# AVianEco/Softspoken

Hardware: AMD Instinct MI355X
Metric: audio-seconds processed/sec (whole node), 16 kHz mono (higher is better)
Workload: dtype f16x2

## Files before the change

### softspoken_amd/csrc/conv4.hip

```cpp
#include "kernels.h"
#include <cstdio>
#include <cstdlib>
#include <type_traits>
#include <utility>

namespace ss {

#ifdef SS_DEVBUILD
static int dev_env(const char* name, int dflt) { const char* v = getenv(name); return v ? atoi(v) : dflt; }
#else
static constexpr int dev_env(const char*, int dflt) { return dflt; }
#endif

typedef float f32x16 __attribute__((ext_vector_type(16)));
typedef float f32x4 __attribute__((ext_vector_type(4)));
typedef float f32x2 __attribute__((ext_vector_type(2)));
typedef __bf16 bf16x8 __attribute__((ext_vector_type(8)));
typedef __bf16 bf16x2 __attribute__((ext_vector_type(2)));
typedef _Float16 f16x8 __attribute__((ext_vector_type(8)));
typedef _Float16 f16x2 __attribute__((ext_vector_type(2)));
typedef short s16x2 __attribute__((ext_vector_type(2)));
typedef uint32_t u32x4 __attribute__((ext_vector_type(4)));
typedef uint32_t u32x2 __attribute__((ext_vector_type(2)));

// ... 5 lines not shown

__device__ __forceinline__ void lds_barrier4() { asm volatile("s_waitcnt lgkmcnt(0)\n\ts_barrier" ::: "memory"); }

__device__ __forceinline__ uint32_t pack_bf16(float lo, float hi) {
    return __builtin_bit_cast(uint32_t, __builtin_convertvector(f32x2{lo, hi}, bf16x2));
}
__device__ __forceinline__ uint32_t relu_pk(uint32_t v) {
    return __builtin_bit_cast(uint32_t, __builtin_elementwise_max(__builtin_bit_cast(s16x2, v), s16x2{0, 0}));
}
__device__ __forceinline__ uint32_t max_pk(uint32_t a, uint32_t b) {
    return __builtin_bit_cast(uint32_t, __builtin_elementwise_max(__builtin_bit_cast(s16x2, a), __builtin_bit_cast(s16x2, b)));
}
__device__ __forceinline__ uint32_t pack_f16(float lo, float hi) {
    return __builtin_bit_cast(uint32_t, __builtin_convertvector(f32x2{lo, hi}, f16x2));
}
__device__ __forceinline__ f32x2 unpack_f16(uint32_t v) { return __builtin_convertvector(__builtin_bit_cast(f16x2, v), f32x2); }
__device__ __forceinline__ uint32_t pk_max_u16(uint32_t a, uint32_t b) {
    uint32_t r;
    asm("v_pk_max_u16 %0, %1, %2" : "=v"(r) : "v"(a), "v"(b));
    return r;
}
__device__ __forceinline__ uint32_t split_lo(uint32_t hi, float x0, float x1) {
    uint32_t l;
    asm("v_fma_mixlo_f16 %0, %1, -1.0, %2 op_sel_hi:[1,0,0]" : "=v"(l) : "v"(hi), "v"(x0));
    asm("v_fma_mixhi_f16 %0, %1, -1.0, %2 op_sel:[1,0,0] op_sel_hi:[1,0,0]" : "+v"(l) : "v"(hi), "v"(x1));
    return l;
}
template <bool F16>
__device__ __forceinline__ f32x16 mfma16(const u32x4& a, const u32x4& b, const f32x16& c) {
    if constexpr (F16) return __builtin_amdgcn_mfma_f32_32x32x16_f16(__builtin_bit_cast(f16x8, a), __builtin_bit_cast(f16x8, b), c, 0, 0, 0);
    else return __builtin_amdgcn_mfma_f32_32x32x16_bf16(__builtin_bit_cast(bf16x8, a), __builtin_bit_cast(bf16x8, b), c, 0, 0, 0);
}
__device__ __forceinline__ void half_swap(uint32_t& x, uint32_t& y) {
    const u32x2 r = __builtin_amdgcn_permlane32_swap(x, y, false, false);
    x = r[0]; y = r[1];
}

struct Packed { uint32_t p[4][2]; };

__device__ __forceinline__ void to_runs(Packed& k, u32x4& lo, u32x4& hi) {
    half_swap(k.p[0][0], k.p[1][0]); half_swap(k.p[0][1], k.p[1][1]);
    half_swap(k.p[2][0], k.p[3][0]); half_swap(k.p[2][1], k.p[3][1]);
    lo = u32x4{k.p[0][0], k.p[0][1], k.p[1][0], k.p[1][1]};
    hi = u32x4{k.p[2][0], k.p[2][1], k.p[3][0], k.p[3][1]};
}
__device__ __forceinline__ void from_runs(const u32x4& lo, const u32x4& hi, Packed& k) {
    k.p[0][0] = lo[0]; k.p[0][1] = lo[1]; k.p[1][0] = lo[2]; k.p[1][1] = lo[3];
    k.p[2][0] = hi[0]; k.p[2][1] = hi[1]; k.p[3][0] = hi[2]; k.p[3][1] = hi[3];
    half_swap(k.p[0][0], k.p[1][0]); half_swap(k.p[0][1], k.p[1][1]);
    half_swap(k.p[2][0], k.p[3][0]); half_swap(k.p[2][1], k.p[3][1]);
}

template <int NT, int NW, bool BRES, bool RES, bool RADD, bool POOL, int RP, bool FIRST, bool FLAT, bool PF2, bool SPLIT = false, bool RANK1 = false,
          int NH = 1>
__global__ __launch_bounds__(64 * NW * NH) __attribute__((amdgpu_waves_per_eu((NT <= 2 && !(SPLIT && RES && !BRES && NW == 4 && NH == 1)) ? 4 : 2)))
void conv3x3_v4_kernel(ConvArgs a, int total_tiles, int lds_b_bytes) {
    constexpr int KC = 32;
    constexpr bool DUO = NH > 1;
    static_assert(!DUO || (NT == 1 && NW * NH == 16 && RP == 0 && !FIRST && !FLAT && !PF2), "DUO: the plain A / B launches");
    constexpr bool RING = DUO && !BRES;
    static_assert(!RING || (SPLIT && NH == 4), "RING: f16x2, four 4-wave tiles");
    static_assert(!SPLIT || !PF2, "SPLIT: single-stage prefetch");
    static_assert(!RANK1 || (SPLIT && !RES && !RADD), "RANK1: conv1_1.B in f16x2 mode");
    static_assert(!(FIRST && SPLIT) || RANK1, "FIRST in f16x2 mode: the block's residual is the fp32 rank-1 term");
    static_assert(!FLAT || (NT == 1 && NW == 8 && BRES && (RADD || RP) && !POOL && !FIRST), "FLAT: conv9_1.B");
    static_assert(!PF2 || (BRES && !FIRST), "two-stage prefetch: resident-weight launches");
    static_assert(RP == 0 || (!RES && !RADD && !FIRST), "RP: a B launch that computes the block's projection itself (no r tensor)");
    static_assert(!FIRST || (NT == 1 && BRES && !RES && !RADD), "FIRST: conv1_1.B, one 32 -> 32 chunk, rank-1 residual");
    constexpr int kTapBytes = 2 * NT * 1024;
    constexpr int TAPS = RES ? 10 : 9;
    constexpr int NTHR = 64 * NW;
    constexpr int TH = 2 * NW;
    constexpr int PR = TH + 2;
    constexpr int kA = PR * kRowPitch;
    constexpr int NPA = PR * kPatch * 4;
    constexpr int AIT = (NPA + NTHR - 1) / NTHR;
    constexpr int NPB = (SPLIT ? 2 : 1) * TAPS * kTapBytes / 16;
    constexpr int BIT = BRES ? 1 : (DUO ? (NPB / 2 + NTHR - 1) / NTHR : (NPB + NTHR - 1) / NTHR);
    static_assert(!(RES && (RADD || POOL)), "RES is the A launch; RADD / POOL belong to B launches");
    static_assert(AIT <= 4, "edge flags are packed 8 bits per piece");
    extern __shared__ __attribute__((aligned(16))) char smem[];

    const int half = DUO ? __builtin_amdgcn_readfirstlane((int)threadIdx.x / NTHR) : 0;
    const int tid = DUO ? (int)threadIdx.x % NTHR : (int)threadIdx.x, lane = tid & 63;
    const int wave = __builtin_amdgcn_readfirstlane(tid >> 6);
    const int hh = lane >> 5, m = lane & 31;
    const int py = (m >> 1) & 1, px = (m & 1) | ((m >> 2) << 1);
    char* sA = smem + half * kA;
    const int sb_bytes = RING ? 2 * lds_b_bytes : lds_b_bytes;
    char* sB = smem + NH * kA;
    const int proj_steps = RP ? (a.C0x + a.C1x) / 16 : 0;
    constexpr bool proj_lds = RP > 0 && (BRES || NT == 3 || SPLIT);
    const char* sProj = smem + NH * kA + sb_bytes;
    const int proj_tiles = SPLIT ? a.Cout / 32 : NT;
    const int proj_bank = proj_steps * proj_tiles * 1024;
    const float* sBias = (const float*)(sProj + (proj_lds ? (SPLIT ? 2 : 1) * proj_bank : 0));
    constexpr int FW = 20, FROWS = PR + 3;
    float* sFb = (float*)sBias + 32;
    float* sF = sFb + 32;
    float* sFlat = (float*)sBias + 32;

    const int H = a.H, W = a.W, Cout = a.Cout;
    const int ngroups = Cout / (32 * NT);
    const int nch_r = (a.C0 + a.C1) / KC;
    const int nch = SPLIT ? 2 * nch_r : nch_r;
    const int all_taps = nch_r * TAPS;

    const int xcd = blockIdx.x & 7, local = (int)(blockIdx.x >> 3) * NH + half, gper = (int)(gridDim.x >> 3) * NH;
    const int per = (total_tiles + 7) >> 3;
#ifdef SS_DEVBUILD
    const bool order_seq = !(a.dbg & 512);
#else
    constexpr bool order_seq = !kOrderSideBySide;
#endif
    auto tile_of = [&](int loc, int it) -> int {
        if constexpr (RING) {
            const RingItem r = ring_item(xcd, loc / NH, (int)(gridDim.x >> 3), it, loc % NH, total_tiles / ngroups, ngroups, order_seq);
            return r.pos >= 0 ? r.pos * ngroups + r.g : -1;
        }
        const int idx = loc + it * gper;
        const int t = xcd * per + idx;
        return (idx < per && t < total_tiles) ? t : -1;
    };
    auto tile_at = [&](int it) -> int { return tile_of(local, it); };
    struct Tile { int n, y0, x0, g; };
    auto decode = [&](int t) -> Tile {
        Tile d;
        d.g = t % ngroups; t /= ngroups;
        d.x0 = (t % a.tiles_x) * 16; t /= a.tiles_x;
        d.y0 = (t % a.tiles_y) * TH;
        d.n = t / a.tiles_y;
        return d;
    };

    uint32_t pix_full[AIT], pix_half[AIT], lds_off[AIT], flags = 0;
    const uint32_t part16 = (tid & 3) * 16;
    {
        const int Wh = W >> 1;
#pragma unroll
        for (int it = 0; it < AIT; ++it) {
            const int p = tid + NTHR * it;
            const int pix = p >> 2;
            const int pyy = pix / kPatch, pxx = pix - pyy * kPatch;
            lds_off[it] = pyy * kRowPitch + pxx * kPixPitch + part16;
            pix_full[it] = pyy * W + pxx;
            pix_half[it] = ((pyy + 1) >> 1) * Wh + ((pxx + 1) >> 1);
            const uint32_t f = (pyy == 0 ? 1u : 0u) | (pyy == PR - 1 ? 2u : 0u) | (pxx == 0 ? 4u : 0u) | (pxx == kPatch - 1 ? 8u : 0u) |
                               (p >= NPA ? 16u : 0u);
            flags |= f << (8 * it);
        }
    }
    u32x4 ra0[AIT], ra1[AIT];
    u32x4 rb[BIT];
    float rf = 0.f;
    static_assert(!FIRST || (PR + 2) * FW <= NTHR, "one feature value per thread");

    auto issue_patch = [&](const Tile& d, int ci, u32x4 (&ra)[AIT]) {
        if constexpr (FIRST) {
            if constexpr (SPLIT) { if (ci & 1) return; }
            const int fy = tid / FW, fx = tid - fy * FW;
            const int Y = d.y0 - 2 + fy, X = d.x0 - 2 + fx;
            rf = (tid < (PR + 2) * FW && (unsigned)Y < (unsigned)H && (unsigned)X < (unsigned)W)
                     ? a.rank1_src[((size_t)d.n * H + Y) * W + X] : 0.f;
            return;
        }
        const int ch = (SPLIT ? ci >> 1 : ci) * KC;
        const int64_t plane = (SPLIT && !(ci & 1)) ? a.lo_delta : 0;
        const char* base; uint32_t cs2, toff; bool up;
// ... 65 lines not shown
                    if (p < NPH) v = *(const u32x4*)(wsrc + p * 16);
                    rb[it] = v;
                }
            } else {
                char* dst = sB + (k & 1) * lds_b_bytes + half * (TAPS * kTapBytes);
#pragma unroll
                for (int it = 0; it < BIT; ++it) {
                    const int p = tid + NTHR * it;
                    if (p < NPH) *(u32x4*)(dst + p * 16) = rb[it];
                }
            }
        }
    };

    constexpr int RPH = RP >= 2 ? RP / 2 : RP;
    u32x4 pxh[(SPLIT && RP) ? RPH : 1], pxl[(SPLIT && RP) ? RPH : 1];
    auto issue_proj = [&](const Tile& d, int chunk, auto k0c, auto k1c) {
        constexpr int K0 = decltype(k0c)::value, K1 = decltype(k1c)::value;
        if constexpr (SPLIT && RP > 0 && K1 > K0) {
            const uint32_t t_full = kHdr + ((((uint32_t)d.n * H + d.y0 + 2 * wave) * W + d.x0) * a.C0x) * 2u;
            const uint32_t t_half = kHdr + ((((uint32_t)d.n * (H >> 1) + (d.y0 >> 1) + wave) * (W >> 1) + (d.x0 >> 1)) * a.C1x) * 2u;
            uint32_t zl = 0;
            asm volatile("" : "+v"(zl));
            const uint32_t xf_o = (uint32_t)((py * W + px) * a.C0x + hh * 8) * 2u + zl, xh_o = (uint32_t)((px >> 1) * a.C1x + hh * 8) * 2u + zl;
#pragma unroll
            for (int k = K0; k < K1; ++k) {
                const int sidx = chunk * RP + k, ch = sidx * 16;
                const char* base; uint32_t off;
                if (sidx >= proj_steps) { base = (const char*)a.xp0 - kHdr; off = 0; }
                else if (ch < a.C0x) { base = (const char*)a.xp0 - kHdr; off = t_full + xf_o + ch * 2u; }
                else { base = (const char*)a.xp1 - kHdr; off = t_half + xh_o + (ch - a.C0x) * 2u; }
                pxh[k - K0] = *(const u32x4*)(base + off);
                pxl[k - K0] = *(const u32x4*)(base + a.lo_delta + off);
            }
        }
    };

    int it_tile = 0;
    struct Stage { int ci; Tile d; };
    auto next_stage = [&](const Stage& s0, Stage& n) -> bool {
        n = s0; n.ci = s0.ci + 1;
        if (n.ci == nch) {
            n.ci = 0;
            const int t = tile_at(++it_tile);
            if (t < 0) return false;
            n.d = decode(t);
        }
        return true;
    };
    int my_stages = 0, max_stages = 0;
    if constexpr (DUO) {
        const int l0 = (int)(blockIdx.x >> 3) * NH;
        int n0 = 0, nmine = 0;
        while (tile_of(l0, n0) >= 0) ++n0;
        while (tile_of(l0 + half, nmine) >= 0) ++nmine;
        my_stages = nmine * nch;
        max_stages = n0 * nch;
        if (max_stages == 0) return;
    } else {
        if (tile_at(0) < 0) return;
    }
    Stage cs{0, decode((DUO && my_stages == 0) ? 0 : tile_at(0))}, n1 = cs, n2 = cs;

    if constexpr (BRES || RING) {
        const char* wsrc = (const char*)a.wpk + (RING ? (size_t)ring_g0 * nch_r * 2 * (TAPS * kTapBytes) : 0);
        for (int p = tid; p < lds_b_bytes / 16; p += NTHR) *(u32x4*)(sB + p * 16) = *(const u32x4*)(wsrc + (size_t)p * 16);
    }
    for (int i = tid; i < Cout * (RES ? 2 : 1); i += NTHR)
        ((float*)sBias)[i] = i < Cout ? a.bias[i] : a.res_bias[i - Cout];
    if constexpr (proj_lds)
        for (int p = tid; p < (SPLIT ? 2 : 1) * proj_steps * proj_tiles * 64; p += NTHR) *(u32x4*)((char*)sProj + p * 16) = *(const u32x4*)((const char*)a.proj_w + (size_t)p * 16);
    u32x4 wfirst = {0u, 0u, 0u, 0u}, wr1 = {0u, 0u, 0u, 0u}, wfirst_lo = {0u, 0u, 0u, 0u};
    constexpr int NMT = (PR * kPatch + 31) / 32;
    int pf_off[2], pa_off[2]; uint32_t pflags = 0;
    if constexpr (FIRST) {
        for (int i = tid; i < 32; i += NTHR) sFb[i] = a.first_b[i];
        for (int i = tid; i < FROWS * FW; i += NTHR) sF[i] = 0.f;
        const float* w9 = a.first_w;
        auto wv = [&](int t) { return w9[t * 32 + m]; };
        if constexpr (SPLIT) {
            auto hi2 = [&](float x, float y) { return pack_f16(x, y); };
            auto lo2 = [&](float x, float y) { const f32x2 b = unpack_f16(pack_f16(x, y)); return pack_f16(x - b[0], y - b[1]); };
            if (hh == 0) {
                wfirst = u32x4{hi2(wv(0), wv(1)), hi2(wv(2), 0.f), hi2(wv(3), wv(4)), hi2(wv(5), 0.f)};
                wfirst_lo = u32x4{lo2(wv(0), wv(1)), lo2(wv(2), 0.f), lo2(wv(3), wv(4)), lo2(wv(5), 0.f)};
            } else {
                wfirst = u32x4{hi2(wv(6), wv(7)), hi2(wv(8), 0.f), 0u, 0u};
                wfirst_lo = u32x4{lo2(wv(6), wv(7)), lo2(wv(8), 0.f), 0u, 0u};
            }
        } else if (hh == 0) {
            wfirst = u32x4{pack_bf16(wv(0), wv(1)), pack_bf16(wv(2), 0.f), pack_bf16(wv(3), wv(4)), pack_bf16(wv(5), 0.f)};
            const float w = a.rank1_w[m];
            const float whi = (float)(__bf16)w, wlo = w - whi;
            wr1 = u32x4{pack_bf16(whi, whi), pack_bf16(wlo, 0.f), 0u, 0u};
        } else {
            wfirst = u32x4{pack_bf16(wv(6), wv(7)), pack_bf16(wv(8), 0.f), 0u, 0u};
        }
#pragma unroll
        for (int t = 0; t < 2; ++t) {
            const int q = 32 * (wave + NW * t) + m;
            const bool in = q < PR * kPatch;
            const int qq = in ? q : 0;
            const int qy = qq / kPatch, qx = qq - qy * kPatch;
            pf_off[t] = (qy + 2 * hh) * FW + qx;
            pa_off[t] = qy * kRowPitch + qx * kPixPitch + hh * 16;
            const uint32_t f = (qy == 0 ? 1u : 0u) | (qy == PR - 1 ? 2u : 0u) | (qx == 0 ? 4u : 0u) | (qx == kPatch - 1 ? 8u : 0u) | (in ? 0u : 16u);
            pflags |= f << (8 * t);
        }
    }
    u32x4 hk_lo[(FIRST && SPLIT) ? 2 : 1], hk_hi[(FIRST && SPLIT) ? 2 : 1];
    auto produce = [&](const Tile& d, int part) {
        const uint32_t tm = (d.y0 == 0 ? 1u : 0u) | (d.y0 + TH == H ? 2u : 0u) | (d.x0 == 0 ? 4u : 0u) | (d.x0 + 16 == W ? 8u : 0u) | 16u;
#pragma unroll
        for (int t = 0; t < 2; ++t) {
            if (wave + NW * t < NMT) {
                if constexpr (SPLIT) {
                    if (part) {
// ... 169 lines not shown
                else { base = (const char*)a.xp1 - kHdr; off = t_half + xh_off + (ch - a.C0x) * 2u; }
                xf[k] = *(const u32x4*)(base + off);
            }
        }
        u32x4 wpg[(RP && !proj_lds) ? RP : 1][NT];
        if constexpr (RP > 0 && !proj_lds && !SPLIT) {
            {
                const int tiles = Cout / 32;
#pragma unroll
                for (int k = 0; k < RP; ++k) {
                    const int sidx = ci * RP + k < proj_steps ? ci * RP + k : 0;
#pragma unroll
                    for (int nt = 0; nt < NT; ++nt)
                        wpg[k][nt] = *(const u32x4*)((const char*)a.proj_w + ((size_t)(sidx * tiles + cur.g * NT + nt) * 64 + lane) * 16);
                }
            }
        }
        if (ci == 0) {
#pragma unroll
            for (int nt = 0; nt < NT; ++nt)
#pragma unroll
                for (int g = 0; g < 4; ++g) {
                    const f32x4 b4 = *(const f32x4*)(sBias + co0 + nt * 32 + 8 * g + 4 * hh);
                    acc[nt][4 * g] = b4[0]; acc[nt][4 * g + 1] = b4[1]; acc[nt][4 * g + 2] = b4[2]; acc[nt][4 * g + 3] = b4[3];
                    if constexpr (RES) {
                        const f32x4 r4 = *(const f32x4*)(sBias + Cout + co0 + nt * 32 + 8 * g + 4 * hh);
                        racc[nt][4 * g] = r4[0]; racc[nt][4 * g + 1] = r4[1]; racc[nt][4 * g + 2] = r4[2]; racc[nt][4 * g + 3] = r4[3];
                    }
                }
        }
        auto proj_products = [&](auto k0c, auto k1c) {
            constexpr int K0 = decltype(k0c)::value, K1 = decltype(k1c)::value;
#pragma unroll
            for (int k = K0; k < K1; ++k) {
                const int sidx = (ci >> 1) * RP + k < proj_steps ? (ci >> 1) * RP + k : 0;
#pragma unroll
                for (int nt = 0; nt < NT; ++nt) {
                    const int wt = (sidx * proj_tiles + (int)(co0 >> 5) + nt) * 1024 + lane * 16;
                    const u32x4 wh = *(const u32x4*)(sProj + wt), wl = *(const u32x4*)(sProj + proj_bank + wt);
                    acc[nt] = mfma16<true>(wh, pxl[k - K0], acc[nt]);
                    acc[nt] = mfma16<true>(wl, pxh[k - K0], acc[nt]);
                    acc[nt] = mfma16<true>(wh, pxh[k - K0], acc[nt]);
                }
            }
        };
        using KZ_ = std::integral_constant<int, 0>; using KH_ = std::integral_constant<int, RPH>; using KR_ = std::integral_constant<int, RP>;
        if constexpr (SPLIT && RP > 0 && PART == 1) {
            proj_products(KZ_{}, KH_{});
            __builtin_amdgcn_sched_barrier(0);
            if constexpr (RP > RPH) issue_proj(cur, ci >> 1, KH_{}, KR_{});
        }
        if constexpr (FLAT && SPLIT && RP > 0) load_flat_w();
        {
            const char* bbase = sB + boff0 + (BRES ? ((DUO ? cur.g * nch : 0) + (SPLIT ? (ci >> 1) * 2 : ci)) * TAPS * kTapBytes
                                                   : RING ? ((stage_no >> 1) & 1) * lds_b_bytes : 0);
            constexpr int PD = (NT == 1) ? 4 : 2;
            u32x4 af[PD], bfr[PD][NT];
            u32x4 rfr[RES ? 2 : 1][RES ? NT : 1];
            if (a.dbg & 32) __builtin_amdgcn_s_setprio(kMfmaPrio);
            constexpr bool kMerged = SPLIT && NSTEP == 36 && NT == 1;
            if constexpr (kMerged) {
                constexpr int PM = 3;
                u32x4 pf[PM], wh_[PM], wl_[PM], rh_[RES ? 2 : 1], rl_[RES ? 2 : 1];
                const char* bb0 = bbase; const char* bb1 = bbase + TAPS * kTapBytes;
                auto load3 = [&](int st, int slot) {
                    const int tap = st >> 1, sub = st & 1, dy = tap / 3, dx = tap % 3;
                    pf[slot] = *(const u32x4*)(sA + aoff0 + dy * kRowPitch + dx * kPixPitch + sub * 32);
                    wh_[slot] = *(const u32x4*)(bb0 + tap * kTapBytes + sub * 1024);
                    wl_[slot] = *(const u32x4*)(bb1 + tap * kTapBytes + sub * 1024);
                };
#pragma unroll
                for (int st = 0; st < PM - 1; ++st) load3(st, st);
#pragma unroll
                for (int st = 0; st < 18; ++st) {
                    if (st + PM - 1 < 18) load3(st + PM - 1, (st + PM - 1) % PM);
                    if constexpr (RES) {
                        if (st == 6) {
#pragma unroll
                            for (int sub = 0; sub < 2; ++sub) {
                                rh_[sub] = *(const u32x4*)(bb0 + 9 * kTapBytes + sub * 1024);
                                rl_[sub] = *(const u32x4*)(bb1 + 9 * kTapBytes + sub * 1024);
                            }
                        }
                    }
                    const u32x4 pixv = pf[st % PM];
                    acc[0] = mfma16<true>(wh_[st % PM], pixv, acc[0]);
                    acc[0] = mfma16<true>(wl_[st % PM], pixv, acc[0]);
                    if constexpr (RES) {
                        if (st == 8 || st == 9) {
                            racc[0] = mfma16<true>(rh_[st & 1], pixv, racc[0]);
                            racc[0] = mfma16<true>(rl_[st & 1], pixv, racc[0]);
                        }
                    }
                }
            } else
#pragma unroll
            for (int bank = 0; bank < NSTEP / 18; ++bank) {
                const char* bb = bbase + bank * TAPS * kTapBytes;
                auto load_frags = [&](int st, u32x4& fa, u32x4 (&fbb)[NT]) {
                    const int tap = st >> 1, sub = st & 1, dy = tap / 3, dx = tap % 3;
                    fa = *(const u32x4*)(sA + aoff0 + dy * kRowPitch + dx * kPixPitch + sub * 32);
#pragma unroll
                    for (int nt = 0; nt < NT; ++nt) fbb[nt] = *(const u32x4*)(bb + tap * kTapBytes + (sub * NT + nt) * 1024);
                };
                if (bank) __builtin_amdgcn_sched_barrier(0);
#pragma unroll
                for (int st = 0; st < PD - 1; ++st) load_frags(st, af[st], bfr[st]);
// ... 228 lines not shown
    #pragma unroll
                            for (int h = 0; h < 2; ++h) {
                                uint32_t v = k.p[g][h];
                                v = max_pk(v, (uint32_t)__builtin_amdgcn_mov_dpp((int)v, 0xB1, 0xf, 0xf, true));
                                v = max_pk(v, (uint32_t)__builtin_amdgcn_mov_dpp((int)v, 0x4E, 0xf, 0xf, true));
                                kp.p[g][h] = v;
                            }
                    }
                    u32x4 lo, hi;
                    if (!FLAT || a.store_out) {
                        to_runs(k, lo, hi);
                        *(u32x4*)(op + nt * 64) = lo;
                        *(u32x4*)(op + nt * 64 + 32) = hi;
                    }
                    if constexpr (RES) {
                        Packed kr;
    #pragma unroll
                        for (int g = 0; g < 4; ++g)
    #pragma unroll
                            for (int h = 0; h < 2; ++h) kr.p[g][h] = pack_bf16(racc[nt][4 * g + 2 * h], racc[nt][4 * g + 2 * h + 1]);
                        to_runs(kr, lo, hi);
                        char* rp = (char*)a.res_out + (o_tile + st_off);
                        *(u32x4*)(rp + nt * 64) = lo;
                        *(u32x4*)(rp + nt * 64 + 32) = hi;
                    }
                    if constexpr (POOL) {
                        to_runs(kp, lo, hi);
                        const u32x4 pv = (m & 1) ? hi : lo;
                        if ((m & 3) < 2) {
                            const uint32_t p_tile = ((((uint32_t)cur.n * (H >> 1) + (cur.y0 >> 1) + wave) * (W >> 1) + (cur.x0 >> 1)) * Cout + co0) * 2u;
                            char* pp = (char*)a.pool_out + (p_tile + pl_off);
                            *(u32x4*)(pp + nt * 64 + (m & 1) * 32) = pv;
                        }
                    }
                }
            }
        };
        constexpr bool EPI_EARLY = PF2;
        jitter(1);
        if constexpr (EPI_EARLY) epilogue();
        lds_barrier4();
        jitter(2);
#ifdef SS_DEVBUILD
        uint32_t tw_i = 0;
#endif
        if constexpr (DUO) {
            if (ok1) {
                commit(ra_a, kCommitPatch, kCommitBank);
                ok2 = next_stage(n1, n2);
                if (ok2) { issue_patch(n2.d, n2.ci, ra_a); issue_weights(n2.d, n2.ci); }
            }
            ring_duty(stage_no, max_stages >> 1);
            ++stage_no;
            jitter(4);
            epilogue();
            jitter(6);
            lds_barrier4();
            jitter(5);
            cs = n1; n1 = n2;
            const bool more = ok1;
            ok1 = ok1 && ok2;
            return more;
        }
        if constexpr (FLAT) { if (flat_pending) flat_reduce(flat_tile); }
        if (ok1) {
            if constexpr (FIRST) {
                if constexpr (!SPLIT || NEXT == 0) {
                    if (tid < (PR + 2) * FW) sF[tid] = rf;
                    lds_barrier4();
                }
                jitter(3);
                produce(n1.d, NEXT);
            } else {
#ifdef SS_DEVBUILD
                uint32_t tw0 = 0;
                if (a.stamps) { tw0 = (uint32_t)__builtin_amdgcn_s_memtime(); asm volatile("s_waitcnt vmcnt(0)" ::: "memory"); const uint32_t t = (uint32_t)__builtin_amdgcn_s_memtime(); st_sum[5] += t - tw0; tw0 = t; }
#endif
                commit(ra_a, kCommitPatch, kCommitBank);
#ifdef SS_DEVBUILD
                if (a.stamps) { asm volatile("s_waitcnt lgkmcnt(0)" ::: "memory"); const uint32_t t = (uint32_t)__builtin_amdgcn_s_memtime(); st_sum[6] += t - tw0; tw_i = t; }
#endif
            }
            if constexpr (PF2) {
                ok3 = ok2 && next_stage(n2, n3);
                if (ok3) issue_patch(n3.d, n3.ci, ra_a);
            } else {
                ok2 = next_stage(n1, n2);
#ifdef SS_DEVBUILD
                if (a.stamps) { const uint32_t t = (uint32_t)__builtin_amdgcn_s_memtime(); st_sum[7] += t - tw_i; tw_i = t; }
#endif
                if (ok2) issue_patch(n2.d, n2.ci, ra_a);
#ifdef SS_DEVBUILD
                if (a.stamps) { const uint32_t t = (uint32_t)__builtin_amdgcn_s_memtime(); st_sum[8] += t - tw_i; tw_i = t;
                                const uint32_t t2 = (uint32_t)__builtin_amdgcn_s_memtime(); st_sum[9] += t2 - t; }
#endif
            }
            if (ok2) issue_weights(n2.d, n2.ci);
            if constexpr (SPLIT && RP > 0 && PART == 0) issue_proj(cur, ci >> 1, KZ_{}, KH_{});
            jitter(4);
            lds_barrier4();
        } else if constexpr (FLAT) {
            lds_barrier4();
        }
        jitter(5);
        if constexpr (!EPI_EARLY) epilogue();
        if constexpr (FLAT) { flat_pending = last; flat_tile = cur; }
        if (!ok1) {
            if constexpr (FLAT) { lds_barrier4(); if (flat_pending) flat_reduce(flat_tile); }
            return false;
        }
        cs = n1; n1 = n2; ok1 = ok2;
        if constexpr (PF2) { n2 = n3; ok2 = ok3; }
        return true;
    };
    using P0 = std::integral_constant<int, 0>; using P1 = std::integral_constant<int, 1>;
    if constexpr (DUO) {
        for (int i = 0; i < half; ++i) lds_barrier4();
        for (int s = 0; s < max_stages; s += SPLIT ? 2 : 1) {
            if (s < my_stages) {
                stage(P0{}, ra0);
                if constexpr (SPLIT) stage(P1{}, ra0);
            } else {
                lds_barrier4(); ring_duty(s, max_stages >> 1); lds_barrier4();
                if constexpr (SPLIT) { lds_barrier4(); ring_duty(s + 1, max_stages >> 1); lds_barrier4(); }
            }
        }
        for (int i = half; i < NH - 1; ++i) lds_barrier4();
    } else if constexpr (SPLIT) {
        while (stage(P0{}, ra0) && stage(P1{}, ra0)) {}
    } else if constexpr (PF2) {
        while (stage(P0{}, ra0) && stage(P0{}, ra1)) {}
    } else {
        while (stage(P0{}, ra0)) {}
    }
#ifdef SS_DEVBUILD
    if (a.stamps && lane == 0) {
        uint32_t* p = (uint32_t*)a.stamps + (((size_t)blockIdx.x * NH + half) * NW + wave) * 16;
        for (int i = 0; i < 5; ++i) p[i] = st_sum[i];
        p[5] = (uint32_t)jit_n; p[6] = st_sum[5]; p[7] = st_sum[6]; p[8] = st_sum[7]; p[9] = st_sum[8]; p[10] = st_sum[9]; p[11] = st_sum[10]; p[12] = st_sum[11];
    }
#endif
}

template <int NT, int NW, bool BRES, bool RES, bool RADD, bool POOL, int RP, bool FIRST, bool FLAT, bool PF2, bool SPLIT = false, bool RANK1 = false,
          int NH = 1>
static hipError_t launch_v4_k(const ConvArgs& a, int total, int lds_b, size_t lds, int grid, hipStream_t s) {
    static std::atomic<uint64_t> attr_done{0};
    if (hipError_t e = allow_full_lds((const void*)conv3x3_v4_kernel<NT, NW, BRES, RES, RADD, POOL, RP, FIRST, FLAT, PF2, SPLIT, RANK1, NH>, attr_done)) return e;
    hipLaunchKernelGGL((conv3x3_v4_kernel<NT, NW, BRES, RES, RADD, POOL, RP, FIRST, FLAT, PF2, SPLIT, RANK1, NH>), dim3(grid), dim3(64 * NW * NH),
                       lds, s, a, total, lds_b);
    return hipGetLastError();
}

template <int NW, int NH, bool BRES>
static hipError_t launch_v4_duo(const ConvArgs& a, int total, int lds_b, size_t lds, int grid, hipStream_t s) {
    if constexpr (BRES && NH == 4) {
        if (a.plain) return launch_v4_k<1, NW, true, false, false, false, 0, false, false, false, true, false, NH>(a, total, lds_b, lds, grid, s);
    }
    if (a.res_out) return launch_v4_k<1, NW, BRES, true, false, false, 0, false, false, false, true, false, NH>(a, total, lds_b, lds, grid, s);
    if (a.pool_out) return launch_v4_k<1, NW, BRES, false, true, true, 0, false, false, false, true, false, NH>(a, total, lds_b, lds, grid, s);
    return launch_v4_k<1, NW, BRES, false, true, false, 0, false, false, false, true, false, NH>(a, total, lds_b, lds, grid, s);
}

template <int NT, int NW>
static hipError_t launch_v4_split(const ConvArgs& a, bool bres, int total, int lds_b, size_t lds, int grid, hipStream_t s) {
    if constexpr (NT == 1 && NW == 8) {
        if (a.rank1_src && a.first_w) return launch_v4_k<1, 8, true, false, false, true, 0, true, false, false, true, true>(a, total, lds_b, lds, grid, s);
        if (a.rank1_src) return launch_v4_k<1, 8, true, false, false, true, 0, false, false, false, true, true>(a, total, lds_b, lds, grid, s);
        if (a.flat_part && a.proj_w) return launch_v4_k<1, 8, true, false, false, false, 4, false, true, false, true>(a, total, lds_b, lds, grid, s);
        if (a.flat_part) return launch_v4_k<1, 8, true, false, true, false, 0, false, true, false, true>(a, total, lds_b, lds, grid, s);
        if (a.proj_w) return bres ? hipErrorInvalidValue : launch_v4_k<1, 8, false, false, false, true, 1, false, false, false, true>(a, total, lds_b, lds, grid, s);
    }
    if (a.res_out) return bres ? launch_v4_k<NT, NW, true, true, false, false, 0, false, false, false, true>(a, total, lds_b, lds, grid, s)
                               : launch_v4_k<NT, NW, false, true, false, false, 0, false, false, false, true>(a, total, lds_b, lds, grid, s);
    if (a.pool_out) return bres ? launch_v4_k<NT, NW, true, false, true, true, 0, false, false, false, true>(a, total, lds_b, lds, grid, s)
                                : launch_v4_k<NT, NW, false, false, true, true, 0, false, false, false, true>(a, total, lds_b, lds, grid, s);
    return bres ? launch_v4_k<NT, NW, true, false, true, false, 0, false, false, false, true>(a, total, lds_b, lds, grid, s)
                : launch_v4_k<NT, NW, false, false, true, false, 0, false, false, false, true>(a, total, lds_b, lds, grid, s);
}

static bool v4_pf2(bool bres, size_t lds, int NT, bool first, bool flat) {
    static const int env = dev_env("SOFTSPOKEN_PF2", 1);
    return env && bres && !first && !flat && NT <= 2 && lds * 3 > 160 * 1024;
}

template <int NT, int NW, bool BRES, bool RES, bool RADD, bool POOL, int RP = 0, bool FIRST = false, bool FLAT = false>
static hipError_t launch_v4_t(const ConvArgs& a, int total, int lds_b, size_t lds, int grid, hipStream_t s) {
    if constexpr (BRES && !FIRST && !FLAT && RP == 0 && NT <= 2 && NW == 8 && !(RES && NT == 2)) {
        if (v4_pf2(true, lds, NT, false, false)) return launch_v4_k<NT, NW, BRES, RES, RADD, POOL, RP, FIRST, FLAT, true>(a, total, lds_b, lds, grid, s);
    }
    return launch_v4_k<NT, NW, BRES, RES, RADD, POOL, RP, FIRST, FLAT, false>(a, total, lds_b, lds, grid, s);
}

static int v4_rp(const ConvArgs& a) {
    if (!a.proj_w) return 0;
    const int steps = (a.C0x + a.C1x) / 16, nch = (a.C0 + a.C1) / 32;
    const int per = (steps + nch - 1) / nch;
    return per <= 1 ? 1 : per <= 2 ? 2 : per <= 4 ? 4 : per <= 6 ? 6 : -1;
}

template <int NT, int NW>
static hipError_t launch_v4_kind(const ConvArgs& a, bool bres, int total, int lds_b, size_t lds, int grid, hipStream_t s) {
    const int rp = v4_rp(a);
    if constexpr (NT == 1 && NW == 8) {
        if (a.first_w) return launch_v4_t<1, 8, true, false, false, true, 0, true>(a, total, lds_b, lds, grid, s);
        if (a.flat_part) return rp == 4 ? launch_v4_t<1, 8, true, false, false, false, 4, false, true>(a, total, lds_b, lds, grid, s)
                                        : launch_v4_t<1, 8, true, false, true, false, 0, false, true>(a, total, lds_b, lds, grid, s);
    }
    if (rp) {
        if constexpr (NT == 2 && NW == 8) { if (bres && a.pool_out && rp == 1) return launch_v4_t<2, 8, true, false, false, true, 1>(a, total, lds_b, lds, grid, s); }
        if constexpr (NT == 3 && NW == 8) { if (!bres && a.pool_out && rp == 2) return launch_v4_t<3, 8, false, false, false, true, 2>(a, total, lds_b, lds, grid, s); }
        if constexpr (NT == 2 && NW == 8) { if (!bres && a.pool_out && rp == 2) return launch_v4_t<2, 8, false, false, false, true, 2>(a, total, lds_b, lds, grid, s); }
        if constexpr (NT == 1 && NW == 4) { if (!bres && !a.pool_out && rp == 2) return launch_v4_t<1, 4, false, false, false, false, 2>(a, total, lds_b, lds, grid, s); }
        if constexpr (NT == 2 && NW == 8) { if (bres && !a.pool_out && rp == 6) return launch_v4_t<2, 8, true, false, false, false, 6>(a, total, lds_b, lds, grid, s); }
        return hipErrorInvalidValue;
    }
    if (a.plain) return bres ? launch_v4_t<NT, NW, true, false, false, false>(a, total, lds_b, lds, grid, s)
                             : launch_v4_t<NT, NW, false, false, false, false>(a, total, lds_b, lds, grid, s);
    if (a.res_out) return bres ? launch_v4_t<NT, NW, true, true, false, false>(a, total, lds_b, lds, grid, s)
                               : launch_v4_t<NT, NW, false, true, false, false>(a, total, lds_b, lds, grid, s);
    if (a.pool_out) return bres ? launch_v4_t<NT, NW, true, false, true, true>(a, total, lds_b, lds, grid, s)
                                : launch_v4_t<NT, NW, false, false, true, true>(a, total, lds_b, lds, grid, s);
    return bres ? launch_v4_t<NT, NW, true, false, true, false>(a, total, lds_b, lds, grid, s)
                : launch_v4_t<NT, NW, false, false, true, false>(a, total, lds_b, lds, grid, s);
}

#ifndef SS_RPROJ_DEFAULT
#define SS_RPROJ_DEFAULT 2
#endif
#ifndef SS_DUO_DEFAULT
#define SS_DUO_DEFAULT 4
#endif
struct V4Choice { bool ok; int nw, total, lds_b, grid; bool bres; size_t lds; int duo; };

static V4Choice choose_v4(ConvArgs& a, int NT, int num_cus, int prec) {
    V4Choice c{};
    if (prec != 1 && prec != 2) return c;
    const bool split = prec == 2;
    if (!a.relu || a.R0 || a.R1) return c;
    const bool first = a.first_w != nullptr, flat = a.flat_part != nullptr, proj = a.proj_w != nullptr;
    const bool rank1 = split && a.rank1_src != nullptr;
    if (split) {
        if (a.lo_delta <= 0) return c;
        static const int rproj_env = dev_env("SOFTSPOKEN_RPROJ", SS_RPROJ_DEFAULT);
        if (proj && !(NT == 1 && a.H % 16 == 0 && ((flat && v4_rp(a) == 4 && rproj_env == 2) || (!flat && a.pool_out && a.Cout == 64 && v4_rp(a) == 1)))) return c;
        if (first && !rank1) return c;
        if (rank1 && !(NT == 1 && a.rank1_w && a.pool_out && !a.res_out && !a.res_in && !flat && a.C0 == 32 && a.C1 == 0 && a.H % 16 == 0)) return c;
        if (NT == 2 || !(NT == 1 || (a.H % 16 == 0))) return c;
    }
    const int rp = v4_rp(a);
    if (flat && !(NT == 1 && a.Cout == 32 && a.C0 == 32 && a.C1 == 0 && a.H % 16 == 0 && a.flat_w4 && (a.res_in || rp == 4) && !a.pool_out && !first)) return c;
    if (first) {
        if (!(NT == 1 && a.Cout == 32 && a.C0 == 32 && a.C1 == 0 && a.H % 16 == 0 && a.first_b && a.rank1_src && a.rank1_w && a.pool_out &&
              !a.res_out && !a.res_in && !proj && !a.plain)) return c;
    } else if (proj) {
        if (a.rank1_src || a.res_out || a.res_in || a.plain || rp < 0 || !a.xp0 || a.C0x % 16 || a.C1x % 16 || (a.C1x && !a.xp1)) return c;
        if (a.C0 != a.Cout || a.C1 != 0) return c;
        if ((double)a.N * a.H * a.W * std::max(a.C0x, a.C1x) * 2.0 + kHdr >= 4294967296.0) return c;
    } else if (a.plain) {
        if (a.rank1_src || a.res_out || a.res_in || a.pool_out) return c;
    } else if (!rank1) {
        if (a.rank1_src) return c;
        if (!(a.res_out || a.res_in) || (a.res_out && (a.res_in || a.pool_out))) return c;
    }
    if (a.W % 16 != 0 || a.H % 8 != 0 || a.Cout % (32 * NT) != 0 || NT < 1 || NT > 3) return c;
    if (a.C0 % 32 || a.C1 % 32 || (a.C1 && ((a.H | a.W) & 1))) return c;
    if ((double)a.N * a.H * a.W * std::max(a.Cout, std::max(a.C0, a.C1)) * 2.0 + kHdr >= 4294967296.0) return c;
    c.nw = (a.H % 16 == 0) ? 8 : 4;
    const int th = 2 * c.nw;
    a.tiles_y = a.H / th; a.tiles_x = a.W / 16;
    const int ngroups = a.Cout / (32 * NT);
    const long total_l = (long)a.N * a.tiles_y * a.tiles_x * ngroups;
    if (total_l <= 0 || total_l > 0x7fffffff) return c;
    c.total = (int)total_l;
    const int tap_bytes = 2 * NT * 1024;
    const int taps = a.res_out ? 10 : 9;
    const int all_taps = ((a.C0 + a.C1) / 32) * taps;
    static const int bres_kb = dev_env("SOFTSPOKEN_BRES_KB", 72);
    const int banks = split ? 2 : 1;
    c.bres = ngroups == 1 && (size_t)all_taps * tap_bytes * banks <= (size_t)((first || flat || rank1) ? 72 : bres_kb) * 1024;
    c.lds_b = c.bres ? all_taps * tap_bytes * banks : taps * tap_bytes * banks;
    if ((first || flat || rank1) && !c.bres) return c;
    if (proj && !flat && !((NT == 2 && c.nw == 8 && c.bres && a.pool_out && rp == 1) ||
                           (NT == 3 && c.nw == 8 && !c.bres && ngroups == 1 && a.pool_out && rp == 2) ||
                           (NT == 2 && c.nw == 8 && !c.bres && ngroups > 1 && a.pool_out && rp == 2) ||
                           (NT == 1 && c.nw == 4 && !c.bres && ngroups > 1 && !a.pool_out && rp == 2) ||
                           (split && NT == 1 && c.nw == 8 && !c.bres && ngroups > 1 && a.pool_out && rp == 1) ||
                           (NT == 2 && c.nw == 8 && c.bres && !a.pool_out && rp == 6)))
        return c;
    static const int duo_env = dev_env("SOFTSPOKEN_DUO", SS_DUO_DEFAULT);
    static const int duo8_env = dev_env("SOFTSPOKEN_DUO_H8", 1);
    if ((duo_env == 2 || duo_env == 4) && split && NT == 1 && (c.nw == 8 || (duo_env == 4 && duo8_env)) && !first && !flat && !proj && !rank1) {
        const int nh = duo_env, thd = 32 / nh;
        const size_t fixed = nh * (size_t)(thd + 2) * kRowPitch + (size_t)a.Cout * 4 * (a.res_out ? 2 : 1);
        const size_t chunk_b = (size_t)taps * tap_bytes * banks;
        const size_t all_b = (size_t)ngroups * all_taps * tap_bytes * banks;
        const bool bres = fixed + all_b <= 160 * 1024;
        static const int ring_env = dev_env("SOFTSPOKEN_RING", 1);
        const bool ring = !bres && nh == 4 && ring_env && (a.res_out != nullptr || ring_env == 2 || (a.H <= 32 && a.res_in != nullptr));
        const size_t lds = fixed + (bres ? all_b : 2 * chunk_b);
        if (((bres && (!a.plain || nh == 4)) || (ring && !a.plain)) && lds <= 160 * 1024) {
            c.duo = nh; c.bres = bres; c.lds_b = (int)(bres ? all_b : chunk_b); c.lds = lds;
            c.nw = 16 / nh;
            a.tiles_y = a.H / thd;
            c.total = (int)((long)a.N * a.tiles_y * a.tiles_x * ngroups);
            c.grid = (num_cus + 7) / 8 * 8;
            if (c.grid * nh > c.total) c.grid = ((c.total + nh - 1) / nh + 7) / 8 * 8;
            c.ok = true;
            return c;
        }
    }
    if (split && a.plain) return c;
    c.lds = (size_t)(th + 2) * kRowPitch + c.lds_b + (size_t)a.Cout * 4 * (a.res_out ? 2 : 1) + (first ? (size_t)(32 + (th + 5) * 20) * 4 : 0) +
            (flat ? (size_t)c.nw * 2 * 64 * 4 : 0) + (proj && (ngroups == 1 || split) ? (size_t)((a.C0x + a.C1x) / 16) * (split ? a.Cout / 32 : NT) * 1024 * banks : 0);
    int bpc = (int)((160 * 1024) / c.lds);
    if (bpc < 1) return c;
    if (bpc > 3) bpc = 3;
    { static const int cap = dev_env("SOFTSPOKEN_BPC", 3); if (bpc > cap) bpc = cap; }
    c.grid = num_cus * bpc;
    if (c.grid > c.total) c.grid = c.total;
    c.grid = (c.grid + 7) / 8 * 8;
    c.ok = true;
    return c;
}

int conv_v4_flat_groups() { return 128 / 16; }

bool conv_v4_supports(const ConvArgs& a_in, int NT, int num_cus, int prec) {
    ConvArgs a = a_in;
    return choose_v4(a, NT, num_cus, prec).ok;
}

const char* conv_v4_variant(const ConvArgs& a_in, int NT, int num_cus, int prec) {
    static thread_local char buf[112];
    ConvArgs a = a_in;
    const V4Choice c = choose_v4(a, NT, num_cus, prec);
    if (!c.ok) return "conv3x3_v4_kernel<invalid>";
    auto tf = [](bool b) { return b ? "true" : "false"; };
    const bool res = a.res_out != nullptr, first = a.first_w != nullptr, flat = a.flat_part != nullptr;
    const int rp = v4_rp(a);
    const bool split = prec == 2, rank1 = split && a.rank1_src != nullptr;
    const bool radd = !res && !first && !a.plain && rp == 0 && !rank1;
    const bool pf2 = !split && rp == 0 && c.nw == 8 && !(res && NT == 2) && v4_pf2(c.bres, c.lds, NT, first, flat);
    if (split)
        snprintf(buf, sizeof buf, "conv3x3_v4_kernel<%d, %d, %s, %s, %s, %s, %d, %s, %s, false, true, %s, %d>", NT, c.nw, tf(c.bres), tf(res), tf(radd),
                 tf(!res && a.pool_out), rp, tf(first), tf(flat), tf(rank1), c.duo ? c.duo : 1);
    else
        snprintf(buf, sizeof buf, "conv3x3_v4_kernel<%d, %d, %s, %s, %s, %s, %d, %s, %s, %s, false, false, 1>", NT, c.nw, tf(c.bres), tf(res), tf(radd),
                 tf(!res && a.pool_out), rp, tf(first), tf(flat), tf(pf2));
    return buf;
}

hipError_t launch_conv3x3_v4(const ConvArgs& a_in, int NT, int num_cus, int prec, hipStream_t s) {
    ConvArgs a = a_in;
    const V4Choice c = choose_v4(a, NT, num_cus, prec);
    if (!c.ok) return hipErrorInvalidValue;
    if (prec == 2) {
        if (c.duo == 2) return launch_v4_duo<8, 2, true>(a, c.total, c.lds_b, c.lds, c.grid, s);
        if (c.duo == 4) return c.bres ? launch_v4_duo<4, 4, true>(a, c.total, c.lds_b, c.lds, c.grid, s)
                                      : launch_v4_duo<4, 4, false>(a, c.total, c.lds_b, c.lds, c.grid, s);
        if (c.nw == 8) {
            switch (NT) {
                case 1: return launch_v4_split<1, 8>(a, c.bres, c.total, c.lds_b, c.lds, c.grid, s);
                case 3: return launch_v4_split<3, 8>(a, c.bres, c.total, c.lds_b, c.lds, c.grid, s);
            }
        } else if (NT == 1) return launch_v4_split<1, 4>(a, c.bres, c.total, c.lds_b, c.lds, c.grid, s);
        return hipErrorInvalidValue;
    }
    if (c.nw == 8) {
        switch (NT) {
            case 1: return launch_v4_kind<1, 8>(a, c.bres, c.total, c.lds_b, c.lds, c.grid, s);
            case 2: return launch_v4_kind<2, 8>(a, c.bres, c.total, c.lds_b, c.lds, c.grid, s);
            case 3: return launch_v4_kind<3, 8>(a, c.bres, c.total, c.lds_b, c.lds, c.grid, s);
        }
    } else {
        switch (NT) {
            case 1: return launch_v4_kind<1, 4>(a, c.bres, c.total, c.lds_b, c.lds, c.grid, s);
            case 2: return launch_v4_kind<2, 4>(a, c.bres, c.total, c.lds_b, c.lds, c.grid, s);
            case 3: return launch_v4_kind<3, 4>(a, c.bres, c.total, c.lds_b, c.lds, c.grid, s);
        }
    }
    return hipErrorInvalidValue;
}

}
```

### softspoken_amd/csrc/kernels.h

```cpp
#pragma once
#include <hip/hip_runtime.h>
#include <stdint.h>
#include <atomic>

namespace ss {

inline hipError_t allow_full_lds(const void* kernel, std::atomic<uint64_t>& done) {
    int dev = 0;
    hipError_t e = hipGetDevice(&dev);
    if (e != hipSuccess) return e;
    const uint64_t bit = 1ull << (dev & 63);
    if (done.load(std::memory_order_acquire) & bit) return hipSuccess;
    e = hipFuncSetAttribute(kernel, hipFuncAttributeMaxDynamicSharedMemorySize, 160 * 1024);
    if (e == hipSuccess) done.fetch_or(bit, std::memory_order_release);
    return e;
}

struct ConvArgs {
    const void* src0; const void* src1;
    const void* res0; const void* res1;
    const void* wpk;
    const float* bias;
    const float* rank1_src;
    const float* rank1_w;
    void* out;
    void* pool_out;
    int N, H, W, C0, C1, R0, R1, Cout;
    int relu;
    int tiles_y, tiles_x;
    int dbg;
    const float* first_w; const float* first_b;
    const void* flat_w; float* flat_part;
    int store_out;
    const void* flat_w4;
    void* res_out; const float* res_bias;
    const void* res_in;
    const void* wpk_b; const float* bias_a;
    int plain;
    const void* proj_w;
    const void* xp0; const void* xp1; int C0x, C1x;
    int64_t lo_delta;
    int* range_flag;
    void* stamps;
};
static constexpr bool kOrderSideBySide = true;
struct RingItem { int pos, g; };
__host__ __device__ inline int ring_lim(int xcd, int total_pos) {
    const int per_pos = (total_pos + 7) >> 3, left = total_pos - xcd * per_pos;
    return left < 0 ? 0 : left < per_pos ? left : per_pos;
}
__host__ __device__ inline int ring_group0(int wg, int ngroups, bool seq) { return seq ? 0 : wg % ngroups; }
__host__ __device__ inline int ring_group_step(int G, int ngroups, bool seq) { return seq ? 1 % ngroups : G % ngroups; }
__host__ __device__ inline RingItem ring_item(int xcd, int wg, int G, int item, int tile, int total_pos, int ngroups, bool seq) {
    const int lim = ring_lim(xcd, total_pos);
    int quad, g;
    if (seq) { quad = wg + (item / ngroups) * G; g = item % ngroups; }
    else { const int j = wg + item * G; quad = j / ngroups; g = j - quad * ngroups; }
    const int idx = 4 * quad + tile;
    return RingItem{idx < lim ? xcd * ((total_pos + 7) >> 3) + idx : -1, g};
}
__host__ __device__ inline int ring_items(int xcd, int wg, int G, int tile, int total_pos, int ngroups, bool seq) {
    const int lim = ring_lim(xcd, total_pos);
    const int quads = lim > tile ? (lim - tile + 3) >> 2 : 0;
    if (seq) return quads > wg ? (quads - wg + G - 1) / G * ngroups : 0;
    const int n = quads * ngroups;
    return n > wg ? (n - wg + G - 1) / G : 0;
}

hipError_t launch_conv3x3_v2(const ConvArgs& a, bool bf16, int NT, int num_cus, hipStream_t s);
const char* conv_v2_variant(const ConvArgs& a, bool bf16, int NT, int num_cus);
int conv_v2_flat_groups(bool bf16);
bool conv_v4_supports(const ConvArgs& a, int NT, int num_cus, int prec);
const char* conv_v4_variant(const ConvArgs& a, int NT, int num_cus, int prec);
int conv_v4_flat_groups();
hipError_t launch_conv3x3_v4(const ConvArgs& a, int NT, int num_cus, int prec, hipStream_t s);

bool conv_ups_supports(const ConvArgs& a, int num_cus);
const char* conv_ups_variant();
size_t conv_ups_weight_bytes(int C0, int C1);
hipError_t launch_conv3x3_ups(const ConvArgs& a, int num_cus, hipStream_t s);
bool conv_upsr_supports(const ConvArgs& a, int num_cus);
const char* conv_upsr_variant();
size_t conv_upsr_weight_bytes(int C0, int C1, int Cout);
hipError_t launch_conv3x3_upsr(const ConvArgs& a, int num_cus, hipStream_t s);

bool conv_ups32_supports(const ConvArgs& a, int NT, int MTW, int num_cus);
const char* conv_ups32_variant(int NT, int MTW);
size_t conv_ups32_weight_bytes(int C0, int C1, int Cout);
hipError_t launch_conv3x3_ups32(const ConvArgs& a, int NT, int MTW, int num_cus, hipStream_t s);

bool conv1_stream_supports(const ConvArgs& a);
const char* conv1_stream_variant(const ConvArgs& a, int form);
size_t conv1_stream_weight_bytes();
hipError_t launch_conv1_stream(const ConvArgs& a, int form, int rows_per_unit, int num_cus, hipStream_t s);

struct Head1dWeights { float w1[4][4][3], b1[4], w2[4][4][3], wr[4][4], b2r[4], wo[4], bo, fscale; };
hipError_t launch_mask_head_parts(const float* parts, int n_parts, const float* flat_bias, const Head1dWeights& hw, float* logits,
                                  int N, hipStream_t s);
hipError_t launch_spec_tail(const void* x, int64_t lo_delta, const float* w , const float* bias, float* spec, int N, int prec,
                            hipStream_t s);

static constexpr int kMelLo = 10, kMelHi = 32, kMelPitch = 43;
struct FrontendTables {
    const float4* pretw;
    const float2* w2048;
    const int* mel_start;
    const int* mel_count;
    const int* mel_off;
    const float* mel_w;
    int mel_nw;
    const float* mel_wp;
    int dbg;
    const float2* win2;
    const float2* twt;
    const float2* wkt;
    const float* mel_wq;
    const int* mel_p0;
};
static constexpr int kMelPairsLo = 9, kMelPairsHi = 20, kMelRow = 60;
// ... 40 lines not shown
```

Before: 30560.

## Pin each workgroup to one output-channel group with resident weights in f16x2 B launches

Adds a GRES mode for f16x2 four-tile B launches. Each workgroup is bound to a single output-channel group and keeps only that group's weight bank resident in LDS, instead of all groups' banks or a rotating ring. It adds matching tile scheduling, an arithmetic item count in place of the counting loops, and support for the pooled-projection B launch, where the projection is issued inside the split pass. The aim is to cut LDS weight footprint and streaming so more launches can use resident weights. The cost is a grid that must be a multiple of 8 times the number of groups, which can worsen load balance.

```diff
diff --git a/softspoken_amd/csrc/conv4.hip b/softspoken_amd/csrc/conv4.hip
--- a/softspoken_amd/csrc/conv4.hip
+++ b/softspoken_amd/csrc/conv4.hip
@@ -81,12 +81,14 @@
 }
 
 template <int NT, int NW, bool BRES, bool RES, bool RADD, bool POOL, int RP, bool FIRST, bool FLAT, bool PF2, bool SPLIT = false, bool RANK1 = false,
-          int NH = 1>
+          int NH = 1, bool GRES = false>
 __global__ __launch_bounds__(64 * NW * NH) __attribute__((amdgpu_waves_per_eu((NT <= 2 && !(SPLIT && RES && !BRES && NW == 4 && NH == 1)) ? 4 : 2)))
 void conv3x3_v4_kernel(ConvArgs a, int total_tiles, int lds_b_bytes) {
     constexpr int KC = 32;
     constexpr bool DUO = NH > 1;
-    static_assert(!DUO || (NT == 1 && NW * NH == 16 && RP == 0 && !FIRST && !FLAT && !PF2), "DUO: the plain A / B launches");
+    static_assert(!DUO || (NT == 1 && NW * NH == 16 && (RP == 0 || (GRES && RP == 1 && POOL)) && !FIRST && !FLAT && !PF2),
+                  "DUO: the plain A / B launches; GRES also conv2_1.B's projection in B");
+    static_assert(!GRES || (DUO && BRES && SPLIT && !RES), "GRES: f16x2 B launches with resident banks");
     constexpr bool RING = DUO && !BRES;
     static_assert(!RING || (SPLIT && NH == 4), "RING: f16x2, four 4-wave tiles");
     static_assert(!SPLIT || !PF2, "SPLIT: single-stage prefetch");
@@ -143,6 +145,10 @@
     constexpr bool order_seq = !kOrderSideBySide;
 #endif
     auto tile_of = [&](int loc, int it) -> int {
+        if constexpr (GRES) {
+            const RingItem r = gres_item(xcd, loc / NH, (int)(gridDim.x >> 3), it, loc % NH, total_tiles / ngroups, ngroups, NH);
+            return r.pos >= 0 ? r.pos * ngroups + r.g : -1;
+        }
         if constexpr (RING) {
             const RingItem r = ring_item(xcd, loc / NH, (int)(gridDim.x >> 3), it, loc % NH, total_tiles / ngroups, ngroups, order_seq);
             return r.pos >= 0 ? r.pos * ngroups + r.g : -1;
@@ -314,8 +320,13 @@
     if constexpr (DUO) {
         const int l0 = (int)(blockIdx.x >> 3) * NH;
         int n0 = 0, nmine = 0;
-        while (tile_of(l0, n0) >= 0) ++n0;
-        while (tile_of(l0 + half, nmine) >= 0) ++nmine;
+        if constexpr (GRES) {
+            n0 = gres_items(xcd, (int)(blockIdx.x >> 3), (int)(gridDim.x >> 3), 0, total_tiles / ngroups, ngroups, NH);
+            nmine = gres_items(xcd, (int)(blockIdx.x >> 3), (int)(gridDim.x >> 3), half, total_tiles / ngroups, ngroups, NH);
+        } else {
+            while (tile_of(l0, n0) >= 0) ++n0;
+            while (tile_of(l0 + half, nmine) >= 0) ++nmine;
+        }
         my_stages = nmine * nch;
         max_stages = n0 * nch;
         if (max_stages == 0) return;
@@ -324,7 +335,10 @@
     }
     Stage cs{0, decode((DUO && my_stages == 0) ? 0 : tile_at(0))}, n1 = cs, n2 = cs;
 
-    if constexpr (BRES || RING) {
+    if constexpr (GRES) {
+        const char* wsrc = (const char*)a.wpk + (size_t)gres_group((int)(blockIdx.x >> 3), ngroups) * nch_r * 2 * (TAPS * kTapBytes);
+        for (int p = (int)threadIdx.x; p < lds_b_bytes / 16; p += NTHR * NH) *(u32x4*)(sB + p * 16) = *(const u32x4*)(wsrc + (size_t)p * 16);
+    } else if constexpr (BRES || RING) {
         const char* wsrc = (const char*)a.wpk + (RING ? (size_t)ring_g0 * nch_r * 2 * (TAPS * kTapBytes) : 0);
         for (int p = tid; p < lds_b_bytes / 16; p += NTHR) *(u32x4*)(sB + p * 16) = *(const u32x4*)(wsrc + (size_t)p * 16);
     }
@@ -600,7 +614,7 @@
         }
         if constexpr (FLAT && SPLIT && RP > 0) load_flat_w();
         {
-            const char* bbase = sB + boff0 + (BRES ? ((DUO ? cur.g * nch : 0) + (SPLIT ? (ci >> 1) * 2 : ci)) * TAPS * kTapBytes
+            const char* bbase = sB + boff0 + (BRES ? ((DUO && !GRES ? cur.g * nch : 0) + (SPLIT ? (ci >> 1) * 2 : ci)) * TAPS * kTapBytes
                                                    : RING ? ((stage_no >> 1) & 1) * lds_b_bytes : 0);
             constexpr int PD = (NT == 1) ? 4 : 2;
             u32x4 af[PD], bfr[PD][NT];
@@ -935,6 +949,7 @@
             }
             ring_duty(stage_no, max_stages >> 1);
             ++stage_no;
+            if constexpr (SPLIT && RP > 0 && PART == 0) issue_proj(cur, ci >> 1, KZ_{}, KH_{});
             jitter(4);
             epilogue();
             jitter(6);
@@ -1026,17 +1041,24 @@
 }
 
 template <int NT, int NW, bool BRES, bool RES, bool RADD, bool POOL, int RP, bool FIRST, bool FLAT, bool PF2, bool SPLIT = false, bool RANK1 = false,
-          int NH = 1>
+          int NH = 1, bool GRES = false>
 static hipError_t launch_v4_k(const ConvArgs& a, int total, int lds_b, size_t lds, int grid, hipStream_t s) {
     static std::atomic<uint64_t> attr_done{0};
-    if (hipError_t e = allow_full_lds((const void*)conv3x3_v4_kernel<NT, NW, BRES, RES, RADD, POOL, RP, FIRST, FLAT, PF2, SPLIT, RANK1, NH>, attr_done)) return e;
-    hipLaunchKernelGGL((conv3x3_v4_kernel<NT, NW, BRES, RES, RADD, POOL, RP, FIRST, FLAT, PF2, SPLIT, RANK1, NH>), dim3(grid), dim3(64 * NW * NH),
+    if (hipError_t e = allow_full_lds((const void*)conv3x3_v4_kernel<NT, NW, BRES, RES, RADD, POOL, RP, FIRST, FLAT, PF2, SPLIT, RANK1, NH, GRES>, attr_done)) return e;
+    hipLaunchKernelGGL((conv3x3_v4_kernel<NT, NW, BRES, RES, RADD, POOL, RP, FIRST, FLAT, PF2, SPLIT, RANK1, NH, GRES>), dim3(grid), dim3(64 * NW * NH),
                        lds, s, a, total, lds_b);
     return hipGetLastError();
 }
 
-template <int NW, int NH, bool BRES>
+template <int NW, int NH, bool BRES, bool GRES = false>
 static hipError_t launch_v4_duo(const ConvArgs& a, int total, int lds_b, size_t lds, int grid, hipStream_t s) {
+    if constexpr (GRES) {
+        static_assert(NH == 4 && NW == 4, "GRES: four 4-wave tiles");
+        if (a.proj_w) return a.pool_out ? launch_v4_k<1, NW, true, false, false, true, 1, false, false, false, true, false, NH, true>(a, total, lds_b, lds, grid, s)
+                                        : hipErrorInvalidValue;
+        if (a.pool_out) return launch_v4_k<1, NW, true, false, true, true, 0, false, false, false, true, false, NH, true>(a, total, lds_b, lds, grid, s);
+        return launch_v4_k<1, NW, true, false, true, false, 0, false, false, false, true, false, NH, true>(a, total, lds_b, lds, grid, s);
+    }
     if constexpr (BRES && NH == 4) {
         if (a.plain) return launch_v4_k<1, NW, true, false, false, false, 0, false, false, false, true, false, NH>(a, total, lds_b, lds, grid, s);
     }
@@ -1114,7 +1136,10 @@
 #ifndef SS_DUO_DEFAULT
 #define SS_DUO_DEFAULT 4
 #endif
-struct V4Choice { bool ok; int nw, total, lds_b, grid; bool bres; size_t lds; int duo; };
+#ifndef SS_GRES_DEFAULT
+#define SS_GRES_DEFAULT 1
+#endif
+struct V4Choice { bool ok; int nw, total, lds_b, grid; bool bres; size_t lds; int duo; bool gres; };
 
 static V4Choice choose_v4(ConvArgs& a, int NT, int num_cus, int prec) {
     V4Choice c{};
@@ -1173,6 +1198,25 @@
         return c;
     static const int duo_env = dev_env("SOFTSPOKEN_DUO", SS_DUO_DEFAULT);
     static const int duo8_env = dev_env("SOFTSPOKEN_DUO_H8", 1);
+    static const int gres_env = dev_env("SOFTSPOKEN_GRES", SS_GRES_DEFAULT);
+    if (gres_env && duo_env == 4 && split && NT == 1 && ngroups > 1 && !first && !flat && !rank1 && !a.plain && !a.res_out &&
+        (proj ? (a.pool_out && rp == 1 && c.nw == 8) : a.res_in != nullptr) && (c.nw == 8 || duo8_env)) {
+        const int nh = 4, thd = 32 / nh;
+        const size_t group_b = (size_t)all_taps * tap_bytes * banks;
+        const size_t proj_b = proj ? (size_t)((a.C0x + a.C1x) / 16) * (a.Cout / 32) * 1024 * banks : 0;
+        const size_t lds = nh * (size_t)(thd + 2) * kRowPitch + group_b + proj_b + (size_t)a.Cout * 4;
+        const long total_pos = (long)a.N * (a.H / thd) * a.tiles_x;
+        const int grid = total_pos <= 0x7fffffff / ngroups ? gres_grid(num_cus, (int)total_pos, ngroups, nh) : 0;
+        if (lds <= 160 * 1024 && gres_grid_ok(grid, ngroups)) {
+            c.duo = nh; c.gres = true; c.bres = true; c.lds_b = (int)group_b; c.lds = lds;
+            c.nw = 16 / nh;
+            a.tiles_y = a.H / thd;
+            c.total = (int)(total_pos * ngroups);
+            c.grid = grid;
+            c.ok = true;
+            return c;
+        }
+    }
     if ((duo_env == 2 || duo_env == 4) && split && NT == 1 && (c.nw == 8 || (duo_env == 4 && duo8_env)) && !first && !flat && !proj && !rank1) {
         const int nh = duo_env, thd = 32 / nh;
         const size_t fixed = nh * (size_t)(thd + 2) * kRowPitch + (size_t)a.Cout * 4 * (a.res_out ? 2 : 1);
@@ -1215,7 +1259,7 @@
 }
 
 const char* conv_v4_variant(const ConvArgs& a_in, int NT, int num_cus, int prec) {
-    static thread_local char buf[112];
+    static thread_local char buf[128];
     ConvArgs a = a_in;
     const V4Choice c = choose_v4(a, NT, num_cus, prec);
     if (!c.ok) return "conv3x3_v4_kernel<invalid>";
@@ -1226,10 +1270,10 @@
     const bool radd = !res && !first && !a.plain && rp == 0 && !rank1;
     const bool pf2 = !split && rp == 0 && c.nw == 8 && !(res && NT == 2) && v4_pf2(c.bres, c.lds, NT, first, flat);
     if (split)
-        snprintf(buf, sizeof buf, "conv3x3_v4_kernel<%d, %d, %s, %s, %s, %s, %d, %s, %s, false, true, %s, %d>", NT, c.nw, tf(c.bres), tf(res), tf(radd),
-                 tf(!res && a.pool_out), rp, tf(first), tf(flat), tf(rank1), c.duo ? c.duo : 1);
+        snprintf(buf, sizeof buf, "conv3x3_v4_kernel<%d, %d, %s, %s, %s, %s, %d, %s, %s, false, true, %s, %d, %s>", NT, c.nw, tf(c.bres), tf(res), tf(radd),
+                 tf(!res && a.pool_out), rp, tf(first), tf(flat), tf(rank1), c.duo ? c.duo : 1, tf(c.gres));
     else
-        snprintf(buf, sizeof buf, "conv3x3_v4_kernel<%d, %d, %s, %s, %s, %s, %d, %s, %s, %s, false, false, 1>", NT, c.nw, tf(c.bres), tf(res), tf(radd),
+        snprintf(buf, sizeof buf, "conv3x3_v4_kernel<%d, %d, %s, %s, %s, %s, %d, %s, %s, %s, false, false, 1, false>", NT, c.nw, tf(c.bres), tf(res), tf(radd),
                  tf(!res && a.pool_out), rp, tf(first), tf(flat), tf(pf2));
     return buf;
 }
@@ -1239,6 +1283,7 @@
     const V4Choice c = choose_v4(a, NT, num_cus, prec);
     if (!c.ok) return hipErrorInvalidValue;
     if (prec == 2) {
+        if (c.gres) return launch_v4_duo<4, 4, true, true>(a, c.total, c.lds_b, c.lds, c.grid, s);
         if (c.duo == 2) return launch_v4_duo<8, 2, true>(a, c.total, c.lds_b, c.lds, c.grid, s);
         if (c.duo == 4) return c.bres ? launch_v4_duo<4, 4, true>(a, c.total, c.lds_b, c.lds, c.grid, s)
                                       : launch_v4_duo<4, 4, false>(a, c.total, c.lds_b, c.lds, c.grid, s);
diff --git a/softspoken_amd/csrc/kernels.h b/softspoken_amd/csrc/kernels.h
--- a/softspoken_amd/csrc/kernels.h
+++ b/softspoken_amd/csrc/kernels.h
@@ -65,6 +65,26 @@
     if (seq) return quads > wg ? (quads - wg + G - 1) / G * ngroups : 0;
     const int n = quads * ngroups;
     return n > wg ? (n - wg + G - 1) / G : 0;
+}
+
+__host__ __device__ inline bool gres_grid_ok(int grid, int ngroups) { return grid > 0 && ngroups > 0 && grid % (8 * ngroups) == 0; }
+__host__ __device__ inline int gres_grid(int num_cus, int total_pos, int ngroups, int nh) {
+    int G = (num_cus + 7) / 8;
+    if (ngroups <= 0 || G % ngroups) return 0;
+    const int units = (((total_pos + 7) >> 3) + nh - 1) / nh;
+    if (units < G / ngroups) G = (units > 0 ? units : 1) * ngroups;
+    return 8 * G;
+}
+__host__ __device__ inline int gres_group(int wg, int ngroups) { return wg % ngroups; }
+__host__ __device__ inline RingItem gres_item(int xcd, int wg, int G, int item, int tile, int total_pos, int ngroups, int nh) {
+    const int lim = ring_lim(xcd, total_pos), S = G / ngroups;
+    const int idx = (wg / ngroups + item * S) * nh + tile;
+    return RingItem{idx < lim ? xcd * ((total_pos + 7) >> 3) + idx : -1, wg % ngroups};
+}
+__host__ __device__ inline int gres_items(int xcd, int wg, int G, int tile, int total_pos, int ngroups, int nh) {
+    const int lim = ring_lim(xcd, total_pos), S = G / ngroups, s = wg / ngroups;
+    const int units = lim > tile ? (lim - tile + nh - 1) / nh : 0;
+    return units > s ? (units - s + S - 1) / S : 0;
 }
 
 hipError_t launch_conv3x3_v2(const ConvArgs& a, bool bf16, int NT, int num_cus, hipStream_t s);
```

Measured after the change: 31130 (median of 6 runs). +1.9%, better.
